# crockwell/far

Measured on AMD Instinct MI355X. Metric: image-pairs/sec (match+solve+regress) at 640x480, higher is better.
Workload: dtype f32

## Files before the change

far_amd/csrc/abi.hip:

```cpp
#include "common.h"

static thread_local int g_last_hip_error = 0;
void far_record_hip_error(int e) { g_last_hip_error = e; }

extern "C" int far_abi_version(void) { return 8; }
#ifndef FAR_BUILD_ID
#define FAR_BUILD_ID "unknown"
#endif
extern "C" const char* far_build_id(void) { return FAR_BUILD_ID; }
extern "C" int far_last_hip_error(void) { return g_last_hip_error; }

static std::atomic<int> g_tuning[16] = {{3}, {0}, {0}, {0}, {0}, {0}, {0}, {0}, {0}, {0}, {0}, {0}, {0}, {0}, {0}, {0}};
extern "C" int far_set_tuning(int key, int value) {
    if (key < 0 || key >= 16) return FAR_EINVAL;
    g_tuning[key].store(value, std::memory_order_relaxed);
    return FAR_OK;
}
int far_get_tuning(int key) { return (key >= 0 && key < 16) ? g_tuning[key].load(std::memory_order_relaxed) : 0; }

#define FAR_SIDE_STREAMS 4
namespace {
struct SideStreams {
    hipStream_t s[FAR_SIDE_STREAMS];
    hipEvent_t fork[FAR_SIDE_STREAMS], join[FAR_SIDE_STREAMS];
    bool ready = false;
};
struct ThreadSides {
    SideStreams dev[64];
};
thread_local ThreadSides t_sides;
SideStreams* side_streams() {
    SideStreams& d = t_sides.dev[far_current_device()];
    if (d.ready) return &d;
    bool ok = true;
    for (int i = 0; i < FAR_SIDE_STREAMS; ++i) {
        ok = ok && hipStreamCreateWithFlags(&d.s[i], hipStreamNonBlocking) == hipSuccess;
        ok = ok && hipEventCreateWithFlags(&d.fork[i], hipEventDisableTiming) == hipSuccess;
        ok = ok && hipEventCreateWithFlags(&d.join[i], hipEventDisableTiming) == hipSuccess;
    }
    d.ready = ok;
    return ok ? &d : nullptr;
}
}

extern "C" void* far_stream_fork(hipStream_t main, int i) {
    SideStreams* d = side_streams();
    if (!d || i < 0 || i >= FAR_SIDE_STREAMS) return nullptr;
    if (hipEventRecord(d->fork[i], main) != hipSuccess || hipStreamWaitEvent(d->s[i], d->fork[i], 0) != hipSuccess) return nullptr;
    return (void*)d->s[i];
}

extern "C" int far_stream_join(hipStream_t main, int i) {
    SideStreams* d = side_streams();
    if (!d || i < 0 || i >= FAR_SIDE_STREAMS) return FAR_EINVAL;
    if (hipEventRecord(d->join[i], d->s[i]) != hipSuccess || hipStreamWaitEvent(main, d->join[i], 0) != hipSuccess) return far_check_launch();
    return FAR_OK;
}
```

far_amd/csrc/conv_igemm_f16s.hip:

```cpp
#include "common.h"
#include "linear_small.h"
#include <vector>
#include <type_traits>

namespace {

typedef _Float16 f16x8 __attribute__((ext_vector_type(8)));
typedef __attribute__((address_space(1))) const void* gptr_t;
typedef __attribute__((address_space(3))) void* lptr_t;

constexpr int TW = 16;
constexpr int A_PXB = 80;
constexpr int ACT_EXP_DEFAULT = 4;

template <int KS, int MW, int ST>
struct Geo {
    static constexpr int TH = 4 * MW;
    static constexpr int HW = ST * (TW - 1) + KS, HH = ST * (TH - 1) + KS;
    static constexpr int PX = KS == 1 ? 64 * MW : HW * HH;
    static constexpr int ROWB = KS == 1 ? 0 : (HW * A_PXB + 255) / 256 * 256;
    static constexpr int A_PLANE = KS == 1 ? PX * A_PXB : HH * ROWB;
    static constexpr int ITEMS = PX * 4;
    __device__ static constexpr int px_off(int hy, int hx) { return hy * ROWB + hx * A_PXB; }
};
// ... 435 lines not shown
                    v.x = fmaxf(v.x, __builtin_fmaf(v.x, as, ab)); v.y = fmaxf(v.y, __builtin_fmaf(v.y, as, ab));
                    v.z = fmaxf(v.z, __builtin_fmaf(v.z, as, ab)); v.w = fmaxf(v.w, __builtin_fmaf(v.w, as, ab));
                    float* dst = ybase + row_off(b0 + j);
                    if (row_ok(b0 + j)) FAR_K9_STORE4(dst, v);
                }
                __builtin_amdgcn_sched_barrier(0);
            }
        };
        auto tile_up_row = [&]() {
            constexpr int PB = 4;
            const int hc = p.Ho >> 1, wc = p.Wo >> 1;
            const float ry = p.Ho > 1 ? (float)(hc - 1) / (float)(p.Ho - 1) : 0.f;
            const float rx = p.Wo > 1 ? (float)(wc - 1) / (float)(p.Wo - 1) : 0.f;
            const long per = (long)p.Ho * p.Wo;
            const long n0 = pix0 / per;
            const int rem = (int)(pix0 - n0 * per);
            const int Y0 = rem / p.Wo, Xh = rem - Y0 * p.Wo + 16 * h;
            const float sy = ry * (float)Y0;
            const int y0 = (int)sy, y1 = y0 + (y0 < hc - 1 ? 1 : 0);
            const float ly = sy - (float)y0, hy = 1.f - ly;
            const float* top = p.up + (cok ? ((n0 * hc + y0) * (long)wc) * p.Cout + co4 : 0);
            const float* bot = p.up + (cok ? ((n0 * hc + y1) * (long)wc) * p.Cout + co4 : 0);
            const int cstep = cok ? p.Cout : 0;
            auto xsrc = [&](int jj, int& x0, int& x1, float& lx) {
                const float sx = rx * (float)(Xh + jj);
                x0 = (int)sx; x1 = x0 + (x0 < wc - 1 ? 1 : 0); lx = sx - (float)x0;
            };
            float4 T[2][PB], B[2][PB];
            auto issue = [&](int b, float4 (&t)[PB], float4 (&bb)[PB]) {
#pragma unroll
                for (int j = 0; j < PB; ++j) {
                    int x0, x1; float lx;
                    xsrc(b * PB + j, x0, x1, lx);
                    t[j] = *reinterpret_cast<const float4*>(top + x1 * cstep);
                    bb[j] = *reinterpret_cast<const float4*>(bot + x1 * cstep);
                }
            };
            int xprev; float lx0; int x1u;
            xsrc(0, xprev, x1u, lx0);
            float4 a = *reinterpret_cast<const float4*>(top + xprev * cstep), c = *reinterpret_cast<const float4*>(bot + xprev * cstep);
            float4 tprev = a, bprev = c;
            issue(0, T[0], B[0]);
            float* const yrow = ybase + (long)(16 * h) * p.Csub;
#pragma unroll
            for (int b = 0; b < 16 / PB; ++b) {
                if (b + 1 < 16 / PB) issue(b + 1, T[(b + 1) & 1], B[(b + 1) & 1]);
                float4 vv[PB];
#pragma unroll
                for (int j = 0; j < PB; ++j) vv[j] = *reinterpret_cast<const float4*>(lw + (16 * h + b * PB + j) * 128 + 4 * l31);
                if (b == 0) { arrived(a); arrived(c); }
#pragma unroll
                for (int j = 0; j < PB; ++j) { arrived(T[b & 1][j]); arrived(B[b & 1][j]); }
#pragma unroll
                for (int j = 0; j < PB; ++j) {
                    int x0, x1; float lx;
                    xsrc(b * PB + j, x0, x1, lx);
                    const bool adv = x0 != xprev;
                    a.x = adv ? tprev.x : a.x; a.y = adv ? tprev.y : a.y; a.z = adv ? tprev.z : a.z; a.w = adv ? tprev.w : a.w;
                    c.x = adv ? bprev.x : c.x; c.y = adv ? bprev.y : c.y; c.z = adv ? bprev.z : c.z; c.w = adv ? bprev.w : c.w;
                    const float4 tb = T[b & 1][j], td = B[b & 1][j];
                    const float hx = 1.f - lx;
                    float4 v = vv[j];
                    v.x += hy * (hx * a.x + lx * tb.x) + ly * (hx * c.x + lx * td.x);
                    v.y += hy * (hx * a.y + lx * tb.y) + ly * (hx * c.y + lx * td.y);
                    v.z += hy * (hx * a.z + lx * tb.z) + ly * (hx * c.z + lx * td.z);
                    v.w += hy * (hx * a.w + lx * tb.w) + ly * (hx * c.w + lx * td.w);
                    v.x = fmaxf(v.x, __builtin_fmaf(v.x, as, ab)); v.y = fmaxf(v.y, __builtin_fmaf(v.y, as, ab));
                    v.z = fmaxf(v.z, __builtin_fmaf(v.z, as, ab)); v.w = fmaxf(v.w, __builtin_fmaf(v.w, as, ab));
                    if (cok) FAR_K9_STORE4(yrow + (long)(b * PB + j) * p.Csub, v);
                    tprev = tb; bprev = td; xprev = x0;
                }
                __builtin_amdgcn_sched_barrier(0);
            }
        };
        if (UP == 2) tile_up_row();
        else if (UP) tile_up();
        else if (resp) tile_out(std::true_type{});
        else tile_out(std::false_type{});
        asm volatile("s_waitcnt lgkmcnt(0)" ::: "memory");
        if (mt == 0) FAR_K9_STAMP(5);
    }
}

__device__ __forceinline__ float la_elu1(float x) { return x > 0.f ? x + 1.f : __builtin_amdgcn_exp2f(x * 1.44269504088896341f); }

template <bool FULL>
__device__ __forceinline__ void la_kv_pass(const ConvArgs& p, const f32x16 (&acc)[2][4], const float (&sc)[4], const float (&sh)[4],
                                           int lo, int hi, long blk, int head0, int HD, int l31, int h, float act_scale) {
    const float unscale = 1.0f / (act_scale * act_scale), fS = (float)p.kv_valid;
#pragma unroll
    for (int hd = 0; hd < 2; ++hd) {
        f32x16 kv;
#pragma unroll
        for (int r = 0; r < 16; ++r) kv[r] = 0.f;
        float ks = 0.f;
#pragma unroll
        for (int mt = 0; mt < 2; ++mt)
#pragma unroll
            for (int g = 0; g < 2; ++g) {
                float ka[8], vb[8];
#pragma unroll
                for (int i = 0; i < 8; ++i) {
                    const int r = 8 * g + i;
                    ka[i] = la_elu1(acc[mt][2 * hd][r] * sc[2 * hd] + sh[2 * hd]);
                    vb[i] = acc[mt][2 * hd + 1][r] * sc[2 * hd + 1] + sh[2 * hd + 1];
                    if (!FULL) {
                        const int q = 32 * mt + 16 * (r >> 3) + (r & 3) + 8 * ((r >> 2) & 1) + 4 * h;
                        ka[i] = (q >= lo && q < hi) ? ka[i] : 0.f;
                    }
                    ks += ka[i];
                }
                f16x8 ah, al, bh, bl;
                split8(make_float4(ka[0], ka[1], ka[2], ka[3]), make_float4(ka[4], ka[5], ka[6], ka[7]), act_scale, ah, al);
                split8(make_float4(vb[0], vb[1], vb[2], vb[3]), make_float4(vb[4], vb[5], vb[6], vb[7]), act_scale, bh, bl);
                kv = __builtin_amdgcn_mfma_f32_32x32x16_f16(ah, bh, kv, 0, 0, 0);
                kv = __builtin_amdgcn_mfma_f32_32x32x16_f16(ah, bl, kv, 0, 0, 0);
                kv = __builtin_amdgcn_mfma_f32_32x32x16_f16(al, bh, kv, 0, 0, 0);
                __builtin_amdgcn_sched_barrier(0);
            }
        ks += shfl_xor_f(ks, 32);
        if (p.overflow) {
            float chk = 0.f;
#pragma unroll
            for (int r = 0; r < 16; ++r) chk += kv[r];
            if (__any(!(fabsf(chk) <= FLT_MAX)) && (l31 | h) == 0) atomicOr(p.overflow, 1);
        }
        float* o = p.kv_part + ((size_t)blk * HD + (head0 + hd) * 32) * 33;
#pragma unroll
        for (int r = 0; r < 16; ++r) o[((r & 3) + 8 * (r >> 2) + 4 * h) * 33 + l31] = (kv[r] * unscale) / fS;
        if (h == 0) o[l31 * 33 + 32] = ks;
    }
}

__device__ __forceinline__ void la_kv_epilogue(const ConvArgs& p, const f32x16 (&acc)[2][4], long pixw, int cout_w, int lane,
                                               float act_scale) {
    const int l31 = lane & 31, h = lane >> 5;
    if (pixw >= p.npix) return;
    const long img = pixw / p.kv_S;
    const long vl = (long)p.kv_valid - (pixw - img * p.kv_S);
    const int valid = vl > 64 ? 64 : (int)vl;
    const int HD = p.Cout >> 1, head0 = cout_w >> 6;
    float sc[4], sh[4];
#pragma unroll
    for (int nt = 0; nt < 4; ++nt) {
        const int co = cout_w + 32 * nt + l31;
        sc[nt] = p.scale[co] * p.out_mul;
        sh[nt] = p.shift ? p.shift[co] : 0.f;
    }
    const long blk = pixw >> 6;
    if (valid == 64) la_kv_pass<true>(p, acc, sc, sh, 0, 64, blk, head0, HD, l31, h, act_scale);
    else la_kv_pass<false>(p, acc, sc, sh, 0, valid, blk, head0, HD, l31, h, act_scale);
}

constexpr int KV_IMG_BYTES = 8 * 2 * 2 * 1024 + 256 * 4;

__global__ __launch_bounds__(256) void k_kv_blocks_reduce(const float* __restrict__ part, int Sp, int per,
                                                          float* __restrict__ kv, unsigned char* __restrict__ img, float act_scale) {
    const int n = blockIdx.y, e = blockIdx.x * 256 + threadIdx.x;
    if (e >= per) return;
    const int nb = Sp >> 6;
    float s = 0.f;
    const float* src = part + (size_t)n * nb * per + e;
#pragma unroll 8
    for (int g = 0; g < nb; ++g, src += per) s += *src;
    kv[(size_t)n * per + e] = s;
    if (img) {
// ... 142 lines not shown
    const int last_nks = !SPLIT ? 1 : (p.Cin - 32 * (nchunks - 1)) > 16 ? 2 : 1;
    const size_t slab_stride = (size_t)p.nblkY * B_BUF;
    const unsigned char* wsrc = p.w + (size_t)by * B_BUF + tid * 16;
    const int nslab = SPLIT ? ((nchunks - 1) * 2 + last_nks) * TAPS : nchunks * TAPS;
    const int first_last = (nchunks - 1) * 2 * TAPS;
    int pidx = 0, pslot = 0;
    auto prefetch = [&]() {
        unsigned char* dst = Bs + pslot * B_BUF + wave * 1024;
#pragma unroll
        for (int j = 0; j < B_ITERS; ++j)
#if defined(FAR_K9_EXP) && (FAR_K9_EXP & 32)
            if ((pidx & 7) == 0)
#endif
            if ((j + 1) * NTHR * 16 <= B_BUF || j * NTHR * 16 + wave * 1024 < B_BUF)
                __builtin_amdgcn_global_load_lds((gptr_t)(wsrc + j * (NTHR * 16)), (lptr_t)(dst + j * (NTHR * 16)), 16, 0, 0);
        pslot = pslot == 2 ? 0 : pslot + 1;
        const size_t adv = (SPLIT && pidx >= first_last && last_nks == 1) ? 2 * slab_stride : slab_stride;
        ++pidx;
        wsrc += pidx < nslab ? adv : 0;
    };

    int a_off[2];
#pragma unroll
    for (int mt = 0; mt < 2; ++mt) {
        const int mtile = 2 * wm + mt;
        if (KS == 1) a_off[mt] = (32 * mtile + l31) * A_PXB + h * 16;
        else a_off[mt] = G::px_off(ST * (2 * mtile + (l31 >> 4)), ST * (l31 & 15)) + h * 16;
    }
    const int b_off = ((N7 ? 96 : 32 * NTW) * wn + l31) * 32 + ((h ^ ((l31 >> 3) & 1)) * 16);

    f32x16 acc[2][NTW];
#pragma unroll
    for (int mt = 0; mt < 2; ++mt)
#pragma unroll
        for (int nt = 0; nt < NTW; ++nt)
#pragma unroll
            for (int r = 0; r < 16; ++r) acc[mt][nt][r] = 0.f;

    const int* rowpix = nullptr;
    if constexpr (EPI == 1 || EPI == 2) {
        if (p.kv_valid != p.kv_S) {
            int* tab = reinterpret_cast<int*>(smem + A_BUF + 3 * B_BUF);
            if (tid < 64 * MW) {
                const long row = tp.pix0 + tid;
                const long im = row / p.kv_S;
                const int t = (int)(row - im * p.kv_S);
                tab[tid] = (row < p.npix && t < p.kv_valid) ? (int)(im * p.kv_valid + t) : -1;
            }
            __syncthreads();
            rowpix = tab;
        }
    }
    if constexpr (EPI == 3) {
        static_assert(KS == 1 && !UP && !N7, "gather mode is a Linear-mode input form");
        int* tab = reinterpret_cast<int*>(smem + A_BUF + 3 * B_BUF);
        if (tid < 64 * MW) {
            const long row = tp.pix0 + tid;
            int gp = -1;
            if (row < p.npix) {
                const unsigned ww = (unsigned)(p.g_W * p.g_W), urow = (unsigned)row;
                const unsigned w = urow / ww, t = urow - w * ww;
                const unsigned cell = (unsigned)p.g_cell[w], b = (unsigned)p.g_b[w];
                const int cy = (int)(cell / (unsigned)p.g_wc), cx = (int)(cell - (unsigned)cy * (unsigned)p.g_wc);
                const int ky = (int)(t / (unsigned)p.g_W), kx = (int)(t - (unsigned)ky * (unsigned)p.g_W);
                const int y = cy * p.g_stride - p.g_W / 2 + ky, x = cx * p.g_stride - p.g_W / 2 + kx;
                if ((unsigned)y < (unsigned)p.g_Hf && (unsigned)x < (unsigned)p.g_Wf) gp = ((int)b * p.g_Hf + y) * p.g_Wf + x;
            }
            tab[tid] = gp;
        }
        __syncthreads();
        rowpix = tab;
    }

    Stage<ITERS> st;
    int pixv[ITERS];
    if constexpr (KS != 1) stage_pixels<KS, MW, ST, NTHR, ITERS>(pixv, p, tp, tid);
    stage_load<KS, MW, ST, NTHR, ITERS>(st, p, tp, 0, tid, true, rowpix, KS != 1 ? pixv : nullptr);
    prefetch();
    prefetch();
    stage_arrived<2 * B_ITERS>(st);
    stage_store<KS, MW, ST, NTHR, ITERS, SPLIT>(st, As, tid, act_scale);
    FAR_K9_STAMP(1);

    constexpr bool APRE = ITERS <= 3;
    constexpr int NH = APRE ? NTW / 2 : 1;
    constexpr int NGRP = NTW / NH;
    f16x8 ah[2], al[2], ahn[2], aln[2], bh[2][NH], bl[2][NH];
    auto read_a = [&](f16x8 (&xh)[2], f16x8 (&xl)[2], int tap, int ks) {
        const int tapoff = KS == 1 ? 0 : G::px_off(tap / KS, tap % KS);
        const unsigned char* A = As + tapoff + ks * 32;
#pragma unroll
        for (int mt = 0; mt < 2; ++mt) {
            xh[mt] = *reinterpret_cast<const f16x8*>(A + a_off[mt]);
            xl[mt] = *reinterpret_cast<const f16x8*>(A + (SPLIT ? G::A_PLANE : 32) + a_off[mt]);
        }
    };
    auto read_b = [&](int grp, const unsigned char* B) {
        const int half = grp & 1;
#pragma unroll
        for (int q = 0; q < NH; ++q) {
#if defined(FAR_K9_EXP) && (FAR_K9_EXP & 16)
            if (q > 0) { bh[half][q] = bh[half][0]; bl[half][q] = bl[half][0]; continue; }
#endif
            bh[half][q] = *reinterpret_cast<const f16x8*>(B + (grp * NH + q) * 32 * 32);
            bl[half][q] = *reinterpret_cast<const f16x8*>(B + B_PLANE + (grp * NH + q) * 32 * 32);
        }
    };
    auto mma_half = [&](int grp) {
        const int half = grp & 1;
#if defined(FAR_K9_EXP) && (FAR_K9_EXP & 64)
#pragma unroll
        for (int q = 0; q < NH; ++q)
#pragma unroll
            for (int mt = 0; mt < 2; ++mt)
                acc[mt][grp * NH + q][0] += (float)ah[mt][0] * (float)bh[half][q][0] + (float)al[mt][0] * (float)bl[half][q][0];
        return;
#endif
        auto live = [&](int mt, int nt) { return !N7 || (WN == 0 ? !(mt == 1 && nt == 3) : !(mt == 0 && nt == 0)); };
#pragma unroll
        for (int q = 0; q < NH; ++q)
#pragma unroll
            for (int mt = 0; mt < 2; ++mt)
                if (live(mt, grp * NH + q))
                    acc[mt][grp * NH + q] = __builtin_amdgcn_mfma_f32_32x32x16_f16(ah[mt], bh[half][q], acc[mt][grp * NH + q], 0, 0, 0);
        if (SPLIT) {
#pragma unroll
            for (int q = 0; q < NH; ++q)
#pragma unroll
                for (int mt = 0; mt < 2; ++mt)
                    if (live(mt, grp * NH + q))
                        acc[mt][grp * NH + q] = __builtin_amdgcn_mfma_f32_32x32x16_f16(ah[mt], bl[half][q], acc[mt][grp * NH + q], 0, 0, 0);
#pragma unroll
            for (int q = 0; q < NH; ++q)
#pragma unroll
                for (int mt = 0; mt < 2; ++mt)
                    if (live(mt, grp * NH + q))
                        acc[mt][grp * NH + q] = __builtin_amdgcn_mfma_f32_32x32x16_f16(al[mt], bh[half][q], acc[mt][grp * NH + q], 0, 0, 0);
        } else {
#pragma unroll
            for (int q = 0; q < NH; ++q)
#pragma unroll
                for (int mt = 0; mt < 2; ++mt)
                    if (live(mt, grp * NH + q))
                        acc[mt][grp * NH + q] = __builtin_amdgcn_mfma_f32_32x32x16_f16(al[mt], bl[half][q], acc[mt][grp * NH + q], 0, 0, 0);
        }
    };

    int slot = 0;
    for (int chunk = 0; chunk < nchunks; ++chunk) {
        const int nks = !SPLIT ? 1 : chunk == nchunks - 1 ? last_nks : 2;
#pragma unroll
        for (int tap = 0; tap < TAPS; ++tap) {
#pragma unroll
            for (int ks = 0; ks < 2; ++ks) {
                if (ks >= nks) continue;
                const bool first = tap == 0 && ks == 0;
                const bool last = tap == TAPS - 1 && ks == nks - 1;
                const bool after_load = SPLIT ? (tap == LOAD_TAP && ks == 1) || (TAPS > 1 && tap == LOAD_TAP + 1 && ks == 0)
                                              : TAPS > 1 && (tap == LOAD_TAP + 1 || tap == LOAD_TAP + 2);
                if (after_load) asm volatile("s_waitcnt vmcnt(%0)" ::"n"(B_ITERS + 2 * ITERS) : "memory");
                else asm volatile("s_waitcnt vmcnt(%0)" ::"n"(B_ITERS) : "memory");
                asm volatile("s_waitcnt lgkmcnt(0)\n\ts_barrier" ::: "memory");
                const unsigned char* B = Bs + slot * B_BUF + b_off;
                read_b(0, B);
                if (first || !APRE) read_a(ah, al, tap, ks);
                __builtin_amdgcn_sched_barrier(0);
                prefetch();
                if (tap == LOAD_TAP && ks == 0) __builtin_amdgcn_sched_barrier(0);
                if (tap == LOAD_TAP && ks == 0)
                    stage_load<KS, MW, ST, NTHR, ITERS>(st, p, tp, chunk + 1, tid, chunk + 1 < nchunks, rowpix, KS != 1 ? pixv : nullptr);
#pragma unroll
                for (int grp = 0; grp < NGRP; ++grp) {
                    if (grp + 1 < NGRP) read_b(grp + 1, B);
                    if (grp == NGRP - 1 && APRE && !(tap == TAPS - 1 && (ks == 1 || !SPLIT))) {
                        const bool wrap = ks + 1 >= nks;
                        read_a(ahn, aln, wrap ? tap + 1 : tap, wrap ? 0 : 1);
                    }
                    mma_half(grp);
                }
#pragma unroll
                for (int i = 0; i < (N7 ? (SPLIT ? 21 : 14) : (SPLIT ? 6 : 4) * NTW); ++i) {
                    __builtin_amdgcn_sched_group_barrier(0x008, 1, 0);
                    __builtin_amdgcn_sched_group_barrier(0x100, 1, 0);
                    __builtin_amdgcn_sched_group_barrier(0x020, 1, 0);
                    __builtin_amdgcn_sched_group_barrier(0x006, 4, 0);
                }
                __builtin_amdgcn_sched_barrier(0);
                (void)last;
#pragma unroll
                for (int mt = 0; mt < 2; ++mt) if (APRE) { ah[mt] = ahn[mt]; al[mt] = aln[mt]; }
                slot = slot == 2 ? 0 : slot + 1;
            }
        }
        stage_arrived<((SPLIT ? 2 * (TAPS - LOAD_TAP) - 1 : TAPS - LOAD_TAP - 1)) * B_ITERS>(st);
        if (chunk + 1 < nchunks) {
            asm volatile("s_waitcnt lgkmcnt(0)\n\ts_barrier" ::: "memory");
            stage_store<KS, MW, ST, NTHR, ITERS, SPLIT>(st, As, tid, act_scale);
        }
    }
    asm volatile("s_waitcnt vmcnt(0)" ::: "memory");
    FAR_K9_STAMP(2);

    if (p.overflow) {
        float chk = 0.f;
#pragma unroll
        for (int mt = 0; mt < 2; ++mt)
#pragma unroll
            for (int nt = 0; nt < NTW; ++nt)
#pragma unroll
                for (int r = 0; r < 16; ++r) chk += acc[mt][nt][r];
        const bool bad = !(fabsf(chk) <= FLT_MAX);
        if (__any(bad) && lane == 0) atomicOr(p.overflow, 1);
    }
#if defined(FAR_K9_EXP) && (FAR_K9_EXP & 2)
    {
        float t = 0.f;
        for (int mt = 0; mt < 2; ++mt) for (int nt = 0; nt < NTW; ++nt) for (int r = 0; r < 16; ++r) t += acc[mt][nt][r];
        if (t == 123.456f) p.y[0] = t;
        return;
    }
#endif
    ConvArgs pe = p;
    pe.out_mul = out_mul;
    if constexpr (EPI == 2) {
        static_assert(KS == 1 && NW == 2 && NTW == 4 && !UP && !N7, "the apply epilogue is a mode of the 256-column Linear tiles");
        asm volatile("s_waitcnt lgkmcnt(0)\n\ts_barrier" ::: "memory");
        la_apply_epilogue(pe, acc, tp.pix0 + 64 * wm, cout_w, lane, reinterpret_cast<float*>(smem) + wave * (32 * LDW), act_scale);
        return;
    }
    if constexpr (EPI == 1) {
        static_assert(KS == 1 && NW == 2 && NTW == 4 && !UP && !N7, "the K'^T V epilogue is a mode of the 256-column Linear tiles");
        la_kv_epilogue(pe, acc, tp.pix0 + 64 * wm, cout_w, lane, act_scale);
        return;
    }
    if (NTW == 4 && ((p.Cout | p.Csub) & 3) == 0) {
        asm volatile("s_waitcnt lgkmcnt(0)\n\ts_barrier" ::: "memory");
        if constexpr (N7)
            conv_epilogue_wide<KS, NW, UP>(pe, acc, tp, cout_w, wm, wave, lane, reinterpret_cast<float*>(smem) + wave * (32 * 128),
                                           reinterpret_cast<float*>(smem) + MW * NW * (32 * 128), wn == 0 ? 1 : 0,
                                           wn == 0 ? 24 : 0, wn == 0 ? 32 : 8);
        else
            conv_epilogue_wide<KS, NW, UP>(pe, acc, tp, cout_w, wm, wave, lane, reinterpret_cast<float*>(smem) + wave * (32 * 128),
                                           reinterpret_cast<float*>(smem) + MW * NW * (32 * 128));
    } else {
        conv_epilogue<KS, NTW>(pe, acc, tp, cout_w, wm, l31, h);
    }
#ifdef FAR_K9_TIMING
    FAR_K9_STAMP(3);
    asm volatile("s_waitcnt vmcnt(0)" ::: "memory");
    FAR_K9_STAMP(4);
    if (threadIdx.x == 0 && blockIdx.x < 65536) g_k9_stamps[12 * blockIdx.x + 9] = __builtin_amdgcn_s_memrealtime();
#endif
}

template <int KS, int MW, int NW, int NTW, bool SPLIT, int ST, int UP = 0, bool N7 = false, int EPI = 0>
__global__ __launch_bounds__(64 * MW * NW, (ST == 1 ? 2 : 1)) void k_conv(const ConvArgs p) {
    if constexpr (N7) {
        if (((threadIdx.x >> 6) % NW) == 1) conv_body<KS, MW, NW, NTW, SPLIT, ST, UP, N7, 1>(p);
        else conv_body<KS, MW, NW, NTW, SPLIT, ST, UP, N7, 0>(p);
    } else {
        conv_body<KS, MW, NW, NTW, SPLIT, ST, UP, N7, 0, EPI>(p);
    }
}

__global__ void k_absmax_bits(const float* __restrict__ w, long n, unsigned* __restrict__ out) {
    __shared__ unsigned part[256];
    unsigned m = 0;
    for (long i = (long)blockIdx.x * blockDim.x + threadIdx.x; i < n; i += (long)gridDim.x * blockDim.x) {
        const unsigned b = __float_as_uint(fabsf(w[i]));
        m = b > m ? b : m;
    }
    part[threadIdx.x] = m;
    __syncthreads();
    for (int d = 128; d >= 1; d >>= 1) {
        if ((int)threadIdx.x < d && part[threadIdx.x + d] > part[threadIdx.x]) part[threadIdx.x] = part[threadIdx.x + d];
        __syncthreads();
    }
    if (threadIdx.x == 0) atomicMax(out, part[0]);
}
template <int MODE>
__device__ __forceinline__ void write_scales(float amax, float* __restrict__ s) {
    int e = 0;
    if (amax > 0.f && amax <= FLT_MAX) (void)frexpf(amax, &e);
    if (MODE == 0) {
        int w_exp = 14 - e;
        w_exp = w_exp < -60 ? -60 : (w_exp > 60 ? 60 : w_exp);
        s[0] = ldexpf(1.0f, w_exp);
        s[1] = ldexpf(1.0f, -(w_exp + ACT_EXP_DEFAULT));
    } else {
        int ex = 10 - e;
        ex = ex < -100 ? -100 : (ex > 100 ? 100 : ex);
        s[0] = ldexpf(1.0f, ex);
        s[1] = ldexpf(1.0f, ACT_EXP_DEFAULT - ex);
    }
}
constexpr long AMAX_SINGLE_MAX = 1L << 16;

template <int MODE>
__global__ __launch_bounds__(1024) void k_amax_scale_single(const float* __restrict__ w, long n, float* __restrict__ s) {
    __shared__ unsigned part[1024];
    unsigned m = 0;
    const long n4 = n >> 2;
    const float4* w4 = reinterpret_cast<const float4*>(w);
    for (long i = threadIdx.x; i < n4; i += 1024) {
        const float4 v = w4[i];
        const unsigned a = __float_as_uint(fabsf(v.x)), b = __float_as_uint(fabsf(v.y)), c = __float_as_uint(fabsf(v.z)),
                       d = __float_as_uint(fabsf(v.w));
        const unsigned ab = a > b ? a : b, cd = c > d ? c : d, q = ab > cd ? ab : cd;
        m = q > m ? q : m;
    }
    for (long i = (n4 << 2) + threadIdx.x; i < n; i += 1024) {
        const unsigned b = __float_as_uint(fabsf(w[i]));
        m = b > m ? b : m;
    }
    part[threadIdx.x] = m;
    __syncthreads();
    for (int d = 512; d >= 1; d >>= 1) {
        if ((int)threadIdx.x < d && part[threadIdx.x + d] > part[threadIdx.x]) part[threadIdx.x] = part[threadIdx.x + d];
        __syncthreads();
    }
    if (threadIdx.x == 0) write_scales<MODE>(__uint_as_float(part[0]), s);
}

struct AmaxSlot {
    unsigned max_bits, ticket;
};
__device__ AmaxSlot g_amax_slots[1024];

template <int MODE>
__global__ __launch_bounds__(256) void k_amax_scale_multi(const float* __restrict__ w, long n, float* __restrict__ s, int slot) {
    __shared__ unsigned part[256];
    unsigned m = 0;
    const long n4 = n >> 2;
    const float4* w4 = reinterpret_cast<const float4*>(w);
    for (long i = (long)blockIdx.x * 256 + threadIdx.x; i < n4; i += (long)gridDim.x * 256) {
        const float4 v = w4[i];
        const unsigned a = __float_as_uint(fabsf(v.x)), b = __float_as_uint(fabsf(v.y)), c = __float_as_uint(fabsf(v.z)),
                       d = __float_as_uint(fabsf(v.w));
        const unsigned ab = a > b ? a : b, cd = c > d ? c : d, q = ab > cd ? ab : cd;
// ... 113 lines not shown
        __threadfence();
        if (atomicAdd(&sl->ticket, 1u) == gridDim.x - 1) {
            __threadfence();
            const unsigned bits = atomicExch(&sl->max_bits, 0u);
            atomicExch(&sl->ticket, 0u);
            write_scales<0>(__uint_as_float(bits), r.pack_scale);
        }
    }
}

__global__ __launch_bounds__(256) void k_pack_table_images(const PackRow* __restrict__ rows) {
    const PackRow r = rows[blockIdx.y];
    const float wmul = r.pack_scale[0];
    if (r.scale_vec && blockIdx.x == 0)
        for (int co = threadIdx.x; co < r.Cout; co += 256) r.scale_vec[co] = (r.base_scale ? r.base_scale[co] : 1.0f) * r.pack_scale[1];
    const long total = (long)r.taps * r.nchunks * 2 * r.nblkY * r.NT * 2;
    if (blockIdx.x == 0 && threadIdx.x < 16) r.out[(size_t)total * 8 * r.planes + threadIdx.x] = (_Float16)0.f;
    for (long i = (long)blockIdx.x * 256 + threadIdx.x; i < total; i += (long)gridDim.x * 256) {
        long t = i;
        const int s = (int)(t & 1); t >>= 1;
        const int nn = (int)(t % r.NT); t /= r.NT;
        const int by = (int)(t % r.nblkY); t /= r.nblkY;
        const int ks = (int)(t & 1); t >>= 1;
        const int tap = (int)(t % r.taps);
        const int chunk = (int)(t / r.taps);
        const int n = by * r.NT + nn;
        const size_t row = r.planes == 2 ? ((((size_t)(chunk * r.taps + tap) * 2 + ks) * r.nblkY + by) * 2) * r.NT + nn
                                         : ((((size_t)(chunk * r.taps + tap) * r.nblkY + by) * 2 + ks)) * r.NT + nn;
        _Float16* dst = r.out + row * 16 + ((s ^ ((nn >> 3) & 1)) * 8);
        for (int e = 0; e < 8; ++e) {
            const int ch = 32 * chunk + 16 * ks + 8 * s + e;
            float v = 0.f;
            if (n < r.Cout && ch < r.Cin) v = r.w[(long)n * r.s_co + (long)ch * r.s_ci + (long)tap * r.s_tap] * wmul;
            const _Float16 hh = (_Float16)v;
            dst[e] = hh;
            if (r.planes == 2) dst[(size_t)r.NT * 16 + e] = (_Float16)(v - (float)hh);
        }
    }
}

struct TileCfg { int mw, nw, nt; };
inline TileCfg cfg_for(int Cout, int stride) {
    const int pad128 = (Cout + 127) / 128 * 128, pad256 = (Cout + 255) / 256 * 256;
    return (stride == 1 && pad128 < pad256) ? TileCfg{4, 1, 128} : TileCfg{2, 2, 256};
}

template <int KS, int MW, int NW, int NTW, bool SPLIT, int ST = 1, int UP = 0, bool N7 = false, int EPI = 0>
int launch_conv(const ConvArgs& a, dim3 grid, hipStream_t stream) {
    using G = Geo<KS, MW, ST>;
    constexpr int PLANES = SPLIT ? 2 : 1;
    constexpr int smem_loop = PLANES * G::A_PLANE + 3 * 2 * 32 * NTW * NW * 32;
    constexpr int smem_epi = EPI == 2 ? MW * NW * 32 * LDW * 4
                                      : MW * NW * (32 * 128 * 4 + 32 * 4);
    constexpr int smem_need = smem_loop + (EPI != 0 ? 64 * MW * 4 : 0);
    constexpr int smem = smem_need > smem_epi ? smem_need : smem_epi;
    bool cfg_failed = false;
    FAR_ONCE_PER_DEVICE(cfg_failed = hipFuncSetAttribute((const void*)k_conv<KS, MW, NW, NTW, SPLIT, ST, UP, N7, EPI>,
                                                         hipFuncAttributeMaxDynamicSharedMemorySize, smem) != hipSuccess);
    if (cfg_failed) return far_check_launch();
    hipLaunchKernelGGL((k_conv<KS, MW, NW, NTW, SPLIT, ST, UP, N7, EPI>), grid, dim3(64 * MW * NW), smem, stream, a);
    return far_check_launch();
}

template <int KS, bool SPLIT>
int launch_cfg(const TileCfg& c, const ConvArgs& a, dim3 grid, hipStream_t stream, bool small = false) {
    if (KS == 1 && a.up) {
        const bool rowwise = (a.Wo & 31) == 0 && far_get_tuning(13) == 0;
        if (c.mw == 4) return rowwise ? launch_conv<1, 4, 1, 4, SPLIT, 1, 2>(a, grid, stream) : launch_conv<1, 4, 1, 4, SPLIT, 1, 1>(a, grid, stream);
        return rowwise ? launch_conv<1, 2, 2, 4, SPLIT, 1, 2>(a, grid, stream) : launch_conv<1, 2, 2, 4, SPLIT, 1, 1>(a, grid, stream);
    }
    if constexpr (KS == 1) {
        if (c.mw == 2 && small) return launch_conv<1, 1, 2, 4, SPLIT>(a, grid, stream);
        if (c.mw == 4 && small) return launch_conv<1, 2, 1, 4, SPLIT>(a, grid, stream);
    }
    if (c.mw == 4) return launch_conv<KS, 4, 1, 4, SPLIT>(a, grid, stream);
    if constexpr (KS == 3) {
        if (a.nblkY == 1 && a.Cout > 192 && a.Cout <= 224 && ((a.Cout | a.Csub) & 3) == 0 && far_get_tuning(4) == 0)
            return launch_conv<KS, 2, 2, 4, SPLIT, 1, false, true>(a, grid, stream);
    }
    return launch_conv<KS, 2, 2, 4, SPLIT>(a, grid, stream);
}

template <bool SPLIT>
int launch_stride2(const ConvArgs& a, dim3 grid, hipStream_t stream) { return launch_conv<3, 2, 2, 4, SPLIT, 2>(a, grid, stream); }

}

extern "C" {

int far_weight_scale_f32(const float* w, long n, float* scale_out, hipStream_t stream);
int far_conv_pack_view_f32(const float* w, long s_co, long s_ci, long s_tap, int Cin, int Cout, int ksize, int stride, int split,
                           const float* scale_in, void* packed, hipStream_t stream);
int far_conv_pack_view_scaled_f32(const float* w, long s_co, long s_ci, long s_tap, int Cin, int Cout, int ksize, int stride, int split,
                                  const float* scale_in, void* packed, const float* base_scale, float* scale_vec_out,
                                  hipStream_t stream);

size_t far_conv_packed_bytes(int Cin, int Cout, int ksize, int stride, int split) {
    if (Cin <= 0 || Cout <= 0 || (ksize != 1 && ksize != 3) || stride < 1 || stride > 2 || (stride == 2 && ksize != 3)) return 0;
    const int NT = cfg_for(Cout, stride).nt;
    const size_t nchunks = (Cin + 31) / 32, nblkY = (Cout + NT - 1) / NT;
    return (size_t)ksize * ksize * nchunks * nblkY * (split ? 2 : 1) * NT * 64 + 32;
}

int far_conv_pack_f32(const float* w, int Cin, int Cout, int ksize, int stride, int w_exp, int split, void* packed,
                      hipStream_t stream) {
    far_clear_errors();
    if (!w || !packed || far_conv_packed_bytes(Cin, Cout, ksize, stride, split) == 0 || w_exp < -60 || w_exp > 60) return FAR_EINVAL;
    const int NT = cfg_for(Cout, stride).nt;
    const int nchunks = (Cin + 31) / 32, nblkY = (Cout + NT - 1) / NT;
    hipLaunchKernelGGL(k_conv_pack, dim3(512), dim3(256), 0, stream, w, (long)Cin * ksize * ksize, (long)ksize * ksize, 1L, Cin, Cout,
                       ksize * ksize, nchunks, nblkY, NT, split ? 2 : 1, ldexpf(1.0f, w_exp), (const float*)nullptr, (_Float16*)packed);
    return far_check_launch();
}

int far_weight_scale_f32(const float* w, long n, float* scale_out, hipStream_t stream) {
    far_clear_errors();
    if (!w || !scale_out || n <= 0) return FAR_EINVAL;
    if ((reinterpret_cast<uintptr_t>(w) & 15) == 0) {
        launch_amax_scale<0>(w, n, scale_out, stream);
    } else {
        hipMemsetAsync(scale_out, 0, 2 * sizeof(float), stream);
        hipLaunchKernelGGL(k_absmax_bits, dim3(256), dim3(256), 0, stream, w, n, reinterpret_cast<unsigned*>(scale_out));
        hipLaunchKernelGGL(k_pack_scale, dim3(1), dim3(1), 0, stream, scale_out);
    }
    return far_check_launch();
}

int far_conv_pack_view_f32(const float* w, long s_co, long s_ci, long s_tap, int Cin, int Cout, int ksize, int stride, int split,
                           const float* scale_in, void* packed, hipStream_t stream) {
    return far_conv_pack_view_scaled_f32(w, s_co, s_ci, s_tap, Cin, Cout, ksize, stride, split, scale_in, packed, nullptr, nullptr, stream);
}

int far_conv_pack_view_scaled_f32(const float* w, long s_co, long s_ci, long s_tap, int Cin, int Cout, int ksize, int stride, int split,
                                  const float* scale_in, void* packed, const float* base_scale, float* scale_vec_out,
                                  hipStream_t stream) {
    far_clear_errors();
    if (!w || !packed || !scale_in || far_conv_packed_bytes(Cin, Cout, ksize, stride, split) == 0) return FAR_EINVAL;
    const int NT = cfg_for(Cout, stride).nt;
    const int nchunks = (Cin + 31) / 32, nblkY = (Cout + NT - 1) / NT;
    const long items = (long)ksize * ksize * nchunks * 2 * nblkY * NT * 2;
    long blocks = (items + 255) / 256;
    blocks = blocks < 1 ? 1 : (blocks > 512 ? 512 : blocks);
    hipLaunchKernelGGL(k_conv_pack, dim3((unsigned)blocks), dim3(256), 0, stream, w, s_co, s_ci, s_tap, Cin, Cout, ksize * ksize, nchunks, nblkY, NT,
                       split ? 2 : 1, 1.0f, scale_in, (_Float16*)packed, base_scale, scale_vec_out);
    return far_check_launch();
}

int far_conv_pack_auto_f32(const float* w, int Cin, int Cout, int ksize, int stride, int split, void* packed, float* scale_out,
                           hipStream_t stream) {
    far_clear_errors();
    if (!w || !packed || !scale_out || far_conv_packed_bytes(Cin, Cout, ksize, stride, split) == 0) return FAR_EINVAL;
    const long n = (long)Cout * Cin * ksize * ksize;
    const int rc = far_weight_scale_f32(w, n, scale_out, stream);
    if (rc != FAR_OK) return rc;
    return far_conv_pack_view_f32(w, (long)Cin * ksize * ksize, (long)ksize * ksize, 1, Cin, Cout, ksize, stride, split, scale_out,
                                  packed, stream);
}

__global__ void k_grad_scale(float* __restrict__ s) {
    const float amax = s[0];
    int e = 0;
    if (amax > 0.f && amax <= FLT_MAX) (void)frexpf(amax, &e);
    int ex = 10 - e;
    ex = ex < -100 ? -100 : (ex > 100 ? 100 : ex);
    s[0] = ldexpf(1.0f, ex);
    s[1] = ldexpf(1.0f, ACT_EXP_DEFAULT - ex);
}
// ... 270 lines not shown
```

far_amd/flags.py:

```python
import os
from collections import namedtuple

Switch = namedtuple('Switch', 'env module attr off_value neutral scope doc')
SWITCHES = [
    Switch('FAR_NO_WINO', 'far_amd.ops', 'USE_WINO', False, 'parity', 'inference',
           'stride-1 3x3 convolutions on K9 (direct implicit GEMM) instead of K17 (Winograd F(2x2,3x3)); same operator, other summation'),
    Switch('FAR_NO_PAD', 'far_amd.loftr.backbone', 'PAD_CHANNELS', False, 'bitwise', 'inference',
           'the 196-channel backbone maps stored with 196 channels instead of 208 (zero weights for the extra ones: exact zeros)'),
    Switch('FAR_NO_PREFETCH', 'far_amd.loftr.model:LoFTR', 'head_prefetch', False, 'bitwise', 'inference',
           "the head's feature stage computed inside forward_rt_prediction instead of enqueued behind K1"),
    Switch('FAR_NO_SIDE_STREAM', 'far_amd.loftr.model:LoFTR', 'head_side_stream', False, 'bitwise', 'inference',
           "the head's feature stage on the step's own stream behind K1 (rounds 2-5) instead of on a second stream next to K1 and the fine level"),
    Switch('FAR_FPN_STREAM', 'far_amd.loftr.model:LoFTR', 'fpn_side_stream', True, 'bitwise', 'inference',
           "OPT-IN (1 switches it ON; default off): the FPN's fine branch on a side stream next to the coarse transformer and K1 (-0.6 ms per 32 "
           "pairs; off by default because the roofline launch -- K17 208 -> 208 @ 240x320 -- then shares the GPU and its in-step duration "
           "in a kernel trace is no longer its own)"),
    Switch('FAR_NO_GATHER_FUSE', 'far_amd.loftr.stages:FinePreprocess', 'fused_gather', False, 'bitwise', 'inference',
           'FinePreprocess.merge_feat on a materialised window tensor (K3 gather + K9) instead of K9 reading through the match indices'),
    Switch('FAR_NO_KV', 'far_amd.loftr.transformer:LoFTREncoderLayer', 'fused_kv', False, 'parity', 'inference',
           "k, v projections + K5's first half as separate launches instead of K9's k|v epilogue (the K'^T V sum changes order)"),
    Switch('FAR_NO_QAPPLY', 'far_amd.loftr.transformer:LoFTREncoderLayer', 'fused_apply', False, 'parity', 'inference',
           "q projection + K5's second half as separate launches instead of K9's attention-apply epilogue (q no longer stays in split operands)"),
    Switch('FAR_NO_STACK', 'far_amd.loftr.transformer:LocalFeatureTransformer', 'stack_self', False, 'bitwise', 'inference',
           "the two 'self' calls of an encoder layer on the two images separately instead of one call on both"),
    Switch('FAR_NO_BN', 'far_amd.ops', 'USE_HIP_BATCHNORM_TRAIN', False, 'parity', 'training',
           'training-mode BatchNorm on nn.BatchNorm2d + torch activations instead of K19 (tests/test_train_kernels_gpu.py holds K19 to the module)'),
]

ENV_ONLY = {
    'FAR_HIP_LIB': ('load', 'path of another build of libfar_hip.so (tools/ab_build.py: same-box A/B against a git revision); skips the build-id check'),
    'FAR_TUNING': ('load', 'comma-separated key=value pairs handed to far_set_tuning at load time, e.g. FAR_TUNING="10=1,8=1" (keys below)'),
    'FAR_SKIP_ASM_CHECK': ('build', "1: far_amd/build.py does not scan the generated code (K9's asm pixel loads; the LDS-DMA ring rule of every kernel with global_load_lds; the half-register writes of the asm fp16 split) after recompiling"),
    'FAR_EXTRA_HIPCC_FLAGS': ('build', 'extra hipcc flags of an experiment build (-DFAR_WINO_EXP=..., tools/wino_exp.sh); part of the build id'),
    'FAR_COMMIT': ('tools', 'commit stamp tools/collect_profiles.sh / tools/step_floors.py write into the profile files'),
    'FAR_C3_PY_NODE': ('bench', "bench.py --workload c3: the encoder layer's autograd node driven from Python instead of far_enc_layer_fwd / _bwd"),
    'FAR_C3_NO_OVERLAP': ('bench', 'bench.py --workload c3: the layer node without side streams'),
    'FAR_C3_PER_OP': ('bench', 'bench.py --workload c3: one autograd node per operator instead of per layer'),
    'FAR_TORCH_ADAMW': ('bench', 'bench.py --workload c3: torch.optim.AdamW instead of K20'),
    'FAR_CUDNN_BENCHMARK': ('bench', 'bench.py: torch.backends.cudnn.benchmark for the vendor comparison legs'),
}

Tuning = namedtuple('Tuning', 'key default values neutral doc')
TUNING = [
    Tuning(0, 3, (0, 1, 2, 4, 7), 'bitwise', 'bit mask of exact-f32 kernels that stagger wave-slot priorities: 1 k_stats, 2 k_match, 4 k_emm_pv'),
    Tuning(1, 0, (1,), 'parity', 'K1 exact-f32 variant: the other tile shape (another summation order of the row statistics)'),
    Tuning(2, 0, (1,), 'bitwise', 'conf_matrix writer variant A (store pattern)'),
    Tuning(3, 0, (1,), 'bitwise', 'conf_matrix writer variant B (store pattern)'),
    Tuning(4, 0, (1,), 'bitwise', 'K9 without the seven-tile mode / K5 windows on the generic path'),
    Tuning(5, 0, (1, 2, 4), 'bitwise', 'K5 apply: tiles per unit'),
    Tuning(6, 0, (64, 256), 'parity', "K5: tokens per K'^T V chunk (another partial-sum grouping)"),
    Tuning(7, 0, (1,), 'bitwise', 'K9 Linear launches always on full-height tiles'),
    Tuning(8, 0, (1,), 'bitwise', 'K17 splits its operands with the five-instruction split2 instead of v_fma_mix (same values)'),
    Tuning(9, 0, (1,), 'bitwise', 'K17 runs a short last channel block on the full body'),
    Tuning(10, 0, (1,), 'bitwise', "K1's match pass without the tile prescreen"),
    Tuning(11, 0, (1, 2), 'bitwise', "K14's pipeline: 0 = 4 waves / 3 slots / counted waits, two workgroups per CU; 1 = 8 waves / 4 slots / counted, one per CU (round 5's form); 2 = 4 waves / 3 slots / vmcnt(0) per phase (fallback without a wait table)"),
    Tuning(12, 0, (1,), 'parity', "K10's inference form on the exact-f32 matrix instruction instead of split fp16"),
    Tuning(15, 0, (1,), 'bitwise', 'K17: 1 = the multiplying wave group does NOT raise its issue priority (the round-4 kernel)'),
    Tuning(13, 0, (1,), 'bitwise', "K9's FPN-merge epilogue in its generic form everywhere"),
]


def off(env):
    if env not in {s.env for s in SWITCHES}:
        raise KeyError(f'{env} is not a registered far_amd switch (far_amd/flags.py)')
    return os.environ.get(env, '0') not in ('', '0')


def value(env, default=None):
    if env not in ENV_ONLY:
        raise KeyError(f'{env} is not a registered far_amd environment variable (far_amd/flags.py)')
    return os.environ.get(env, default)


def known():
    return {s.env for s in SWITCHES} | set(ENV_ONLY)


def unknown_in_environment():
    skip = ('FAR_WINO_', 'FAR_K9_')
    return sorted(k for k in os.environ if k.startswith('FAR_') and k not in known() and not k.startswith(skip))


def target(sw):
    import importlib
    mod, _, cls = sw.module.partition(':')
    obj = importlib.import_module(mod)
    return (getattr(obj, cls) if cls else obj), sw.attr
```

Before: 381.0.

## Run 3x3 stride-2 conv on eight-wave 64-channel tiles with a dedicated epilogue

The 3x3 stride-2 implicit-GEMM conv now launches by default as 2x4 waves, each covering 64 output channels, instead of 2x2 waves covering 128. A new LDS-staged wide epilogue handles the two-n-tile accumulator, and A-fragment prefetching is enabled for this form. Launch bounds now allow two workgroups per CU. The aim is more waves per SIMD to hide latency, at the cost of more A-operand rereads and register or LDS pressure. Tuning key 16 restores the old four-wave form.

```diff
diff --git a/far_amd/csrc/abi.hip b/far_amd/csrc/abi.hip
--- a/far_amd/csrc/abi.hip
+++ b/far_amd/csrc/abi.hip
@@ -10,13 +10,14 @@
 extern "C" const char* far_build_id(void) { return FAR_BUILD_ID; }
 extern "C" int far_last_hip_error(void) { return g_last_hip_error; }
 
-static std::atomic<int> g_tuning[16] = {{3}, {0}, {0}, {0}, {0}, {0}, {0}, {0}, {0}, {0}, {0}, {0}, {0}, {0}, {0}, {0}};
+static constexpr int N_TUNING = 17;
+static std::atomic<int> g_tuning[N_TUNING] = {{3}, {0}, {0}, {0}, {0}, {0}, {0}, {0}, {0}, {0}, {0}, {0}, {0}, {0}, {0}, {0}, {0}};
 extern "C" int far_set_tuning(int key, int value) {
-    if (key < 0 || key >= 16) return FAR_EINVAL;
+    if (key < 0 || key >= N_TUNING) return FAR_EINVAL;
     g_tuning[key].store(value, std::memory_order_relaxed);
     return FAR_OK;
 }
-int far_get_tuning(int key) { return (key >= 0 && key < 16) ? g_tuning[key].load(std::memory_order_relaxed) : 0; }
+int far_get_tuning(int key) { return (key >= 0 && key < N_TUNING) ? g_tuning[key].load(std::memory_order_relaxed) : 0; }
 
 #define FAR_SIDE_STREAMS 4
 namespace {
diff --git a/far_amd/csrc/conv_igemm_f16s.hip b/far_amd/csrc/conv_igemm_f16s.hip
--- a/far_amd/csrc/conv_igemm_f16s.hip
+++ b/far_amd/csrc/conv_igemm_f16s.hip
@@ -541,6 +541,67 @@
     }
 }
 
+__device__ __forceinline__ void conv_epilogue_wide2(const ConvArgs& p, const f32x16 (&acc)[2][2], const TilePos& tp, int cout_w, int wm,
+                                                    int lane, float* lw) {
+    const int l31 = lane & 31, h = lane >> 5, l15 = lane & 15, prow = lane >> 4;
+    const float* __restrict__ resp = p.res;
+    float* __restrict__ yp = p.y;
+#pragma unroll
+    for (int nt = 0; nt < 2; ++nt) {
+        const int co = cout_w + 32 * nt + l31;
+        const float sc = co < p.Cout ? p.scale[co] * p.out_mul : 0.f;
+        const float sh = (co < p.Cout && p.shift) ? p.shift[co] : 0.f;
+#pragma unroll
+        for (int mt = 0; mt < 2; ++mt)
+#pragma unroll
+            for (int r = 0; r < 16; ++r) {
+                const int q = 32 * mt + 16 * (r >> 3) + (r & 3) + 8 * ((r >> 2) & 1) + 4 * h;
+                lw[q * 64 + 32 * nt + l31] = acc[mt][nt][r] * sc + sh;
+            }
+    }
+    asm volatile("s_waitcnt lgkmcnt(0)" ::: "memory");
+    const int co4 = cout_w + 4 * l15;
+    const bool cok = co4 < p.Cout;
+    const int plane = cok ? co4 / p.Csub : 0;
+    const long cbase = (long)plane * p.npix * p.Csub + (co4 - plane * p.Csub);
+    const int oy = tp.oy0 + 4 * wm;
+    const long pix0 = ((long)tp.img * p.Ho + oy) * p.Wo + tp.ox0;
+    const int nrow = p.Ho - oy, ncol = p.Wo - tp.ox0;
+    const float as = p.act == 2 ? p.slope : 0.f, ab = p.act == 0 ? -__builtin_inff() : 0.f;
+    float* const ybase = yp + (pix0 * (long)p.Csub + cbase);
+    auto row_ok = [&](int it) { return cok && (it >> 2) < nrow && 4 * (it & 3) + prow < ncol; };
+    auto row_off = [&](int it) { return (unsigned)(((it >> 2) * p.Wo + 4 * (it & 3) + prow) * p.Csub); };
+    auto tile_out = [&](auto has_res) {
+        constexpr bool HR = decltype(has_res)::value;
+        float4 rr[16];
+        if (HR) {
+            const float* rbase = resp + (pix0 * (long)p.Csub + cbase);
+#pragma unroll
+            for (int it = 0; it < 16; ++it)
+                rr[it] = *reinterpret_cast<const float4*>(row_ok(it) ? rbase + row_off(it) : resp);
+#pragma unroll
+            for (int it = 0; it < 16; ++it) arrived(rr[it]);
+        }
+#pragma unroll
+        for (int b0 = 0; b0 < 16; b0 += 8) {
+            float4 vv[8];
+#pragma unroll
+            for (int j = 0; j < 8; ++j) vv[j] = *reinterpret_cast<const float4*>(lw + (4 * (b0 + j) + prow) * 64 + 4 * l15);
+#pragma unroll
+            for (int j = 0; j < 8; ++j) {
+                float4 v = vv[j];
+                if (HR) { v.x += rr[b0 + j].x; v.y += rr[b0 + j].y; v.z += rr[b0 + j].z; v.w += rr[b0 + j].w; }
+                v.x = fmaxf(v.x, __builtin_fmaf(v.x, as, ab)); v.y = fmaxf(v.y, __builtin_fmaf(v.y, as, ab));
+                v.z = fmaxf(v.z, __builtin_fmaf(v.z, as, ab)); v.w = fmaxf(v.w, __builtin_fmaf(v.w, as, ab));
+                float* dst = ybase + row_off(b0 + j);
+                if (row_ok(b0 + j)) FAR_K9_STORE4(dst, v);
+            }
+        }
+    };
+    if (resp) tile_out(std::true_type{});
+    else tile_out(std::false_type{});
+}
+
 __device__ __forceinline__ float la_elu1(float x) { return x > 0.f ? x + 1.f : __builtin_amdgcn_exp2f(x * 1.44269504088896341f); }
 
 template <bool FULL>
@@ -849,7 +910,7 @@
     stage_store<KS, MW, ST, NTHR, ITERS, SPLIT>(st, As, tid, act_scale);
     FAR_K9_STAMP(1);
 
-    constexpr bool APRE = ITERS <= 3;
+    constexpr bool APRE = ITERS <= 3 || NTW == 2;
     constexpr int NH = APRE ? NTW / 2 : 1;
     constexpr int NGRP = NTW / NH;
     f16x8 ah[2], al[2], ahn[2], aln[2], bh[2][NH], bl[2][NH];
@@ -1000,17 +1061,28 @@
         la_kv_epilogue(pe, acc, tp.pix0 + 64 * wm, cout_w, lane, act_scale);
         return;
     }
-    if (NTW == 4 && ((p.Cout | p.Csub) & 3) == 0) {
-        asm volatile("s_waitcnt lgkmcnt(0)\n\ts_barrier" ::: "memory");
-        if constexpr (N7)
-            conv_epilogue_wide<KS, NW, UP>(pe, acc, tp, cout_w, wm, wave, lane, reinterpret_cast<float*>(smem) + wave * (32 * 128),
-                                           reinterpret_cast<float*>(smem) + MW * NW * (32 * 128), wn == 0 ? 1 : 0,
-                                           wn == 0 ? 24 : 0, wn == 0 ? 32 : 8);
-        else
-            conv_epilogue_wide<KS, NW, UP>(pe, acc, tp, cout_w, wm, wave, lane, reinterpret_cast<float*>(smem) + wave * (32 * 128),
-                                           reinterpret_cast<float*>(smem) + MW * NW * (32 * 128));
+    const bool wide = ((p.Cout | p.Csub) & 3) == 0;
+    if constexpr (NTW == 4) {
+        if (wide) {
+            asm volatile("s_waitcnt lgkmcnt(0)\n\ts_barrier" ::: "memory");
+            if constexpr (N7)
+                conv_epilogue_wide<KS, NW, UP>(pe, acc, tp, cout_w, wm, wave, lane, reinterpret_cast<float*>(smem) + wave * (32 * 128),
+                                               reinterpret_cast<float*>(smem) + MW * NW * (32 * 128), wn == 0 ? 1 : 0,
+                                               wn == 0 ? 24 : 0, wn == 0 ? 32 : 8);
+            else
+                conv_epilogue_wide<KS, NW, UP>(pe, acc, tp, cout_w, wm, wave, lane, reinterpret_cast<float*>(smem) + wave * (32 * 128),
+                                               reinterpret_cast<float*>(smem) + MW * NW * (32 * 128));
+        } else {
+            conv_epilogue<KS, NTW>(pe, acc, tp, cout_w, wm, l31, h);
+        }
     } else {
-        conv_epilogue<KS, NTW>(pe, acc, tp, cout_w, wm, l31, h);
+        static_assert(NTW == 2 && KS == 3 && !UP && !N7 && EPI == 0, "64-channel wave tiles: the eight-wave form of the 3x3 stride-2 mode");
+        if (wide) {
+            asm volatile("s_waitcnt lgkmcnt(0)\n\ts_barrier" ::: "memory");
+            conv_epilogue_wide2(pe, acc, tp, cout_w, wm, lane, reinterpret_cast<float*>(smem) + wave * (64 * 64));
+        } else {
+            conv_epilogue<KS, NTW>(pe, acc, tp, cout_w, wm, l31, h);
+        }
     }
 #ifdef FAR_K9_TIMING
     FAR_K9_STAMP(3);
@@ -1021,7 +1093,7 @@
 }
 
 template <int KS, int MW, int NW, int NTW, bool SPLIT, int ST, int UP = 0, bool N7 = false, int EPI = 0>
-__global__ __launch_bounds__(64 * MW * NW, (ST == 1 ? 2 : 1)) void k_conv(const ConvArgs p) {
+__global__ __launch_bounds__(64 * MW * NW, ((ST == 1 || MW * NW == 8) ? 2 : 1)) void k_conv(const ConvArgs p) {
     if constexpr (N7) {
         if (((threadIdx.x >> 6) % NW) == 1) conv_body<KS, MW, NW, NTW, SPLIT, ST, UP, N7, 1>(p);
         else conv_body<KS, MW, NW, NTW, SPLIT, ST, UP, N7, 0>(p);
@@ -1301,7 +1373,10 @@
 }
 
 template <bool SPLIT>
-int launch_stride2(const ConvArgs& a, dim3 grid, hipStream_t stream) { return launch_conv<3, 2, 2, 4, SPLIT, 2>(a, grid, stream); }
+int launch_stride2(const ConvArgs& a, dim3 grid, hipStream_t stream) {
+    if (a.ln_gamma || a.post_res || far_get_tuning(16) != 0) return launch_conv<3, 2, 2, 4, SPLIT, 2>(a, grid, stream);
+    return launch_conv<3, 2, 4, 2, SPLIT, 2>(a, grid, stream);
+}
 
 }
 
diff --git a/far_amd/flags.py b/far_amd/flags.py
--- a/far_amd/flags.py
+++ b/far_amd/flags.py
@@ -57,6 +57,7 @@
     Tuning(12, 0, (1,), 'parity', "K10's inference form on the exact-f32 matrix instruction instead of split fp16"),
     Tuning(15, 0, (1,), 'bitwise', 'K17: 1 = the multiplying wave group does NOT raise its issue priority (the round-4 kernel)'),
     Tuning(13, 0, (1,), 'bitwise', "K9's FPN-merge epilogue in its generic form everywhere"),
+    Tuning(16, 0, (1,), 'bitwise', "K9's 3x3 stride-2 mode on its four-wave form (2 x 2 waves, one per SIMD) instead of the eight-wave form"),
 ]
 
 
```

After: 383.1, median of 6. About the same (+0.5%).
